# codelion/adaptive-classifier

Measured on AMD Instinct MI355X. Metric: predict() queries/sec + kNN GB/s vs HBM roofline, 768-d, higher is better.
Workload: dtype f32

## Files before the change

### adaptive-classifier_amd/csrc/attention_core.h

```cpp
#pragma once
#include "common.h"

#include <math.h>

namespace acattn {

typedef float f32x4 __attribute__((ext_vector_type(4)));
typedef float f32x16 __attribute__((ext_vector_type(16)));

__device__ __forceinline__ int crow32(int r, int h) { return (r & 3) + 8 * (r >> 2) + 4 * h; }

__device__ __forceinline__ void rope_rotate(f32x4 (&x)[8], const float* cs, const float* sn, int pos, int h) {
#pragma clang fp contract(off)
#pragma unroll
    for (int kb = 0; kb < 4; ++kb) {
        const f32x4 c = *reinterpret_cast<const f32x4*>(cs + (int64_t)pos * 32 + 8 * kb + 4 * h);
        const f32x4 s = *reinterpret_cast<const f32x4*>(sn + (int64_t)pos * 32 + 8 * kb + 4 * h);
        const f32x4 lo = x[kb], hi = x[kb + 4];
        x[kb] = lo * c + (-hi) * s;
        x[kb + 4] = hi * c + lo * s;
    }
}

template <bool ROPE, int DHT, bool FP32_OUT = true>
__device__ __forceinline__ void attention_tile(const float* qb, const float* kb_, const float* vb, int64_t ld, int S, int qt, int lane,
                                               float scale, const int64_t* mask_row, const float* rope_cos, const float* rope_sin,
                                               int window, float* ctx_rows, int H, uint16_t* ctx_planes, int64_t rows, int64_t row0,
                                               int headcol, int f16) {
#pragma clang fp contract(off)
    static_assert(DHT == 64 || (DHT == 32 && !ROPE), "head dim 64, or 32 without RoPE");
    constexpr int NKB = DHT / 8;
    const int j = lane & 31, h = lane >> 5;
    const int qi = qt * 32 + j;
    const bool qvalid = qi < S;

    f32x4 Qf[NKB];
    {
        const float* qp = qb + (int64_t)(qvalid ? qi : S - 1) * ld + 4 * h;
#pragma unroll
        for (int kb = 0; kb < NKB; ++kb) Qf[kb] = *reinterpret_cast<const f32x4*>(qp + 8 * kb);
        if constexpr (ROPE) rope_rotate(Qf, rope_cos, rope_sin, qvalid ? qi : S - 1, h);
#pragma unroll
        for (int kb = 0; kb < NKB; ++kb) Qf[kb] = Qf[kb] * scale;
    }
    f32x16 o0, o1;
#pragma unroll
    for (int r = 0; r < 16; ++r) { o0[r] = 0.f; o1[r] = 0.f; }
    float m = -INFINITY, l = 0.f;

    f32x4 Kf[NKB];
    auto load_k = [&](int k0) {
        int kr = k0 + j; if (kr > S - 1) kr = S - 1;
        const float* kp = kb_ + (int64_t)kr * ld + 4 * h;
#pragma unroll
        for (int kb = 0; kb < NKB; ++kb) Kf[kb] = *reinterpret_cast<const f32x4*>(kp + 8 * kb);
        if constexpr (ROPE) rope_rotate(Kf, rope_cos, rope_sin, kr, h);
    };
    int kbeg = 0, kend = S;
    if (window >= 0) {
        kbeg = qt * 32 - window; kbeg = kbeg < 0 ? 0 : (kbeg / 32) * 32;
        const int last = qt * 32 + 31 + window;
        if (last + 1 < kend) kend = last + 1;
    }
    load_k(kbeg);
    for (int k0 = kbeg; k0 < kend; k0 += 32) {
        const int kj = k0 + j;
        const bool kv = kj < S && (!mask_row || mask_row[kj] != 0);
        const unsigned vmask = (unsigned)(__ballot(kv && h == 0) & 0xffffffffull);
        if (vmask == 0u) { load_k(k0 + 32); continue; }
        f32x16 st;
#pragma unroll
        for (int r = 0; r < 16; ++r) st[r] = 0.f;
#pragma unroll
        for (int kb = 0; kb < NKB; ++kb)
#pragma unroll
            for (int s4 = 0; s4 < 4; ++s4)
                st = __builtin_amdgcn_mfma_f32_32x32x2f32(Kf[kb][s4], Qf[kb][s4], st, 0, 0, 0);
        load_k(k0 + 32);
        float cmax = -INFINITY;
#pragma unroll
        for (int r = 0; r < 16; ++r) {
            bool ok = (vmask >> crow32(r, h)) & 1u;
            if (window >= 0) { const int dk = qi - (k0 + crow32(r, h)); ok = ok && dk <= window && -dk <= window; }
            st[r] = ok ? st[r] : -INFINITY;
            cmax = fmaxf(cmax, st[r]);
        }
        cmax = fmaxf(cmax, __shfl_xor(cmax, 32));
        const float m_new = fmaxf(m, cmax);
        const bool none = m_new == -INFINITY;
        constexpr float kLog2e = 1.4426950408889634f;
        const float corr = none ? 1.f : __builtin_amdgcn_exp2f((m - m_new) * kLog2e);
        float psum = 0.f;
        float p[16];
#pragma unroll
        for (int r = 0; r < 16; ++r) { p[r] = none ? 0.f : __builtin_amdgcn_exp2f((st[r] - m_new) * kLog2e); psum += p[r]; }
        psum += __shfl_xor(psum, 32);
        l = __builtin_fmaf(l, corr, psum);
        m = m_new;
#pragma unroll
        for (int r = 0; r < 16; ++r) { o0[r] *= corr; o1[r] *= corr; }
#pragma unroll
        for (int r = 0; r < 16; ++r) {
            int vr = k0 + crow32(r, h); if (vr > S - 1) vr = S - 1;
            const float* vp = vb + (int64_t)vr * ld + j;
            o0 = __builtin_amdgcn_mfma_f32_32x32x2f32(vp[0], p[r], o0, 0, 0, 0);
            if constexpr (DHT == 64) o1 = __builtin_amdgcn_mfma_f32_32x32x2f32(vp[32], p[r], o1, 0, 0, 0);
        }
    }
    if (qvalid) {
        const float inv = l > 0.f ? 1.f / l : 0.f;
        if (!FP32_OUT || ctx_planes) {
            const int64_t row = row0 + qi, plane = rows * H;
#pragma unroll
            for (int t = 0; t < DHT / 32; ++t)
#pragma unroll
                for (int g = 0; g < 4; ++g) {
                    f32x4 v;
#pragma unroll
                    for (int e = 0; e < 4; ++e) v[e] = (t ? o1[4 * g + e] : o0[4 * g + e]) * inv;
                    ac::emit_planes4(ctx_planes + ac::plane_off(rows, row, headcol + 32 * t + 8 * g + 4 * h), plane, v, f16);
                }
        } else if constexpr (FP32_OUT) {
            float* dst = ctx_rows + (int64_t)qi * H;
#pragma unroll
            for (int r = 0; r < 16; ++r) {
                dst[crow32(r, h)] = o0[r] * inv;
                if constexpr (DHT == 64) dst[32 + crow32(r, h)] = o1[r] * inv;
            }
        }
    }
}

}
```

### adaptive-classifier_amd/csrc/gemm_pipe.hip

```cpp
#include "common.h"
#include "gemm_common.h"
#include "grid_sync.h"
#include "attention_core.h"

#include <stdio.h>
#include <stdlib.h>

#include <atomic>
#include <type_traits>

namespace {
using namespace acg;

constexpr int PSBK = 16;

struct PipeParams {
    const uint16_t* Ap; int64_t a_rows;
    const uint16_t* Wp; int64_t w_rows;
    float* C; int64_t ldc;
    int M, N, K;
    Epilogue epi;
    LnFuse ln;
    AttnFuse at;
    unsigned long long* stamps;
    int krot;
};

template <int STRIDE = 4>
__device__ __forceinline__ void stamp(const PipeParams& prm, int wave, int i) {
    if (prm.stamps && wave == 0) {
        const unsigned long long t = clock64();
        if ((threadIdx.x & 63) == 0) prm.stamps[(size_t)blockIdx.x * STRIDE + i] = t;
    }
}

template <int N> __device__ __forceinline__ void wait_vm() {
    static_assert(N >= 0 && N <= 63, "vmcnt immediate");
    asm volatile("s_waitcnt vmcnt(%0)" ::"n"(N) : "memory");
}

template <int TM, int TN, int WMW, int WNW, int NS, int AR = 3> struct PipeGeom {
    static constexpr int BM = 32 * TM * WMW, BN = 32 * TN * WNW;
    static constexpr int RA = BM / 32, RW = BN / 32, RG = RA + RW;
    static constexpr int NP = AR * RG;
    static constexpr int NW = WMW * WNW;
    static constexpr int PPW = (NP + NW - 1) / NW;
    static constexpr int SLOT = AR * RG * 64;
    static constexpr int LDS_BYTES = NS * SLOT * 16;
    static constexpr int TR_BYTES = NW * kTrFloats * 4;
    static constexpr int BPC_LDS = (160 * 1024) / (LDS_BYTES > TR_BYTES ? LDS_BYTES : TR_BYTES);
    static constexpr int BPC = BPC_LDS < 1 ? 1 : (BPC_LDS * NW > 16 ? (16 / NW < 1 ? 1 : 16 / NW) : BPC_LDS);
    static constexpr int WAVES_PER_SIMD = (BPC * NW + 3) / 4;
};

template <int TM, int TN, int WMW, int WNW>
__device__ __forceinline__ void ln_prefetch_residual(float (&res)[TM * TN * 16], const PipeParams& prm, int m0, int n0, int wm,
                                                     int wn, int lane) {
#pragma unroll
    for (int mi = 0; mi < TM; ++mi)
#pragma unroll
        for (int ni = 0; ni < TN; ++ni) {
            const int col = n0 + wn * (32 * TN) + ni * 32 + (lane & 31);
            const int64_t rbase = m0 + wm * (32 * TM) + mi * 32;
#pragma unroll
            for (int r = 0; r < 16; ++r) {
                int64_t row = rbase + acc_row32(r, lane);
                if (row > prm.M - 1) row = prm.M - 1;
                res[(mi * TN + ni) * 16 + r] = prm.epi.residual[row * prm.epi.ldr + col];
            }
        }
}

template <int TM, int TN, int WMW, int WNW, int AR>
__device__ __forceinline__ void store_tile_ln(f32x16 (&acc)[TM][TN], const float (&res)[TM * TN * 16], const PipeParams& prm,
                                              int bm, int bn, int ntn, int wm, int wn, int lane, int tid, int wave, float* lds_f) {
    constexpr int BM = 32 * TM * WMW, BN = 32 * TN * WNW, NW = WMW * WNW, WC = 32 * TN;
    static_assert(BM <= 64 * NW, "one thread per tile row in the combine steps");
    const Epilogue& e = prm.epi;
    const LnFuse& ln = prm.ln;
    float2* wstat = reinterpret_cast<float2*>(lds_f + NW * kTrFloats);
    float2* rstat = wstat + WNW * BM;
    unsigned* okf = reinterpret_cast<unsigned*>(rstat + BM);
    const int m0 = bm * BM, n0 = bn * BN, c = lane & 31;
#pragma unroll
    for (int mi = 0; mi < TM; ++mi)
#pragma unroll
        for (int ni = 0; ni < TN; ++ni) {
            const float bias = e.bias[n0 + wn * WC + ni * 32 + c];
#pragma unroll
            for (int r = 0; r < 16; ++r) acc[mi][ni][r] = (acc[mi][ni][r] + bias) + res[(mi * TN + ni) * 16 + r];
        }
#pragma unroll
    for (int mi = 0; mi < TM; ++mi)
#pragma unroll
        for (int r = 0; r < 16; ++r) {
            float s = 0.f;
#pragma unroll
            for (int ni = 0; ni < TN; ++ni) s += acc[mi][ni][r];
            s = acp::row16_sum(s);
            s += __shfl_xor(s, 16);
            const float mw = s * (1.0f / WC);
            float q = 0.f;
#pragma unroll
            for (int ni = 0; ni < TN; ++ni) { const float d = acc[mi][ni][r] - mw; q = fmaf(d, d, q); }
            q = acp::row16_sum(q);
            q += __shfl_xor(q, 16);
            if (c == r) wstat[wn * BM + wm * (32 * TM) + mi * 32 + acc_row32(r, lane)] = make_float2(mw, q);
        }
    __syncthreads();
    if (tid < BM) {
        float mean = 0.f;
#pragma unroll
        for (int w = 0; w < WNW; ++w) mean += wstat[w * BM + tid].x;
        mean *= 1.0f / WNW;
        float m2 = 0.f;
#pragma unroll
        for (int w = 0; w < WNW; ++w) { const float2 pw = wstat[w * BM + tid]; const float d = pw.x - mean; m2 += fmaf((float)WC * d, d, pw.y); }
        const unsigned long long bits = (unsigned long long)__float_as_uint(mean) | ((unsigned long long)__float_as_uint(m2) << 32);
        __hip_atomic_store(reinterpret_cast<unsigned long long*>(ln.part + ((size_t)bm * ntn + bn) * BM + tid), bits,
                           __ATOMIC_RELAXED, __HIP_MEMORY_SCOPE_AGENT);
    }
    asm volatile("s_waitcnt vmcnt(0)" ::: "memory");
    __syncthreads();
    if (tid == 0) {
        if (ln.fences) __hip_atomic_fetch_add(ln.count + bm, 1u, __ATOMIC_RELEASE, __HIP_MEMORY_SCOPE_AGENT);
        else __hip_atomic_fetch_add(ln.count + bm, 1u, __ATOMIC_RELAXED, __HIP_MEMORY_SCOPE_AGENT);
    }
    if (tid < 64) {
        unsigned ok = 1;
        for (long spins = 0;; ++spins) {
            const unsigned v = __hip_atomic_load(ln.count + bm, __ATOMIC_RELAXED, __HIP_MEMORY_SCOPE_AGENT);
            if (v >= (unsigned)(ntn + ln.starve)) {
                if (ln.fences) __builtin_amdgcn_fence(__ATOMIC_ACQUIRE, "agent");
                else asm volatile("" ::: "memory");
                break;
            }
            __builtin_amdgcn_s_sleep(1);
            if ((spins & 63) == 63 && (spins > (1l << 20) || __hip_atomic_load(ln.abort_, __ATOMIC_RELAXED, __HIP_MEMORY_SCOPE_AGENT))) {
                if (lane == 0) __hip_atomic_store(ln.abort_, 1u, __ATOMIC_RELAXED, __HIP_MEMORY_SCOPE_AGENT);
                ok = 0;
                break;
            }
        }
        if (lane == 0) *okf = ok;
    }
    __syncthreads();
    if (tid < BM) {
        float2 pj[8];
        const float* base = reinterpret_cast<const float*>(ln.part + (size_t)bm * ntn * BM + tid);
#pragma unroll
        for (int j = 0; j < 8; ++j) pj[j] = j < ntn ? acp::ld2_sc1(base + (size_t)j * BM * 2) : make_float2(0.f, 0.f);
        float mean = 0.f;
#pragma unroll
        for (int j = 0; j < 8; ++j) mean += pj[j].x;
        mean /= (float)ntn;
        float m2 = 0.f;
#pragma unroll
        for (int j = 0; j < 8; ++j) if (j < ntn) { const float d = pj[j].x - mean; m2 += fmaf((float)BN * d, d, pj[j].y); }
        const float var = m2 / (float)prm.N;
        const float rstd = 1.0f / sqrtf(var + ln.eps);
        rstat[tid] = make_float2(mean, *okf ? rstd : __uint_as_float(0x7fc00000u));
    }
    __syncthreads();
#pragma unroll
    for (int mi = 0; mi < TM; ++mi)
#pragma unroll
        for (int ni = 0; ni < TN; ++ni) {
            const int col = n0 + wn * WC + ni * 32 + c;
            const float g = ln.gamma[col], b = ln.beta[col];
#pragma unroll
            for (int r = 0; r < 16; ++r) {
                const float2 st = rstat[wm * (32 * TM) + mi * 32 + acc_row32(r, lane)];
                acc[mi][ni][r] = (acc[mi][ni][r] - st.x) * st.y * g + b;
            }
        }
    store_tile<EPI_IDENT, TM, BM, TN>(acc, prm.C, prm.ldc, prm.M, prm.N, m0, n0, wm, wn, lane, e);
    if (ln.planes)
        store_tile_planes<EPI_IDENT, TM, TN, AR>(acc, ln.planes, prm.M, prm.N, m0, n0, wm, wn, lane, e, lds_f + wave * kTrFloats);
}

constexpr int kAtLd = 196;
constexpr int kAtRows = 160;
constexpr int kAtCu = ac::kQkvAttnCu;
constexpr int kAtBytes = kAtRows * kAtLd * 4 + kAtCu * 4;

template <int TM, int TN, int WMW, int WNW, int AR>
__device__ __forceinline__ void qkv_attention_epilogue(f32x16 (&acc)[TM][TN], const PipeParams& prm, int bm, int head, int wm, int wn,
                                                       int lane, int wave, float* T, int cu_pref, const float (&bias)[TN]) {
    static_assert(TM == 2 && TN == 3 && WMW == 4 && WNW == 2, "built for the 256 x 192 tile (8 waves of 64 x 96)");
    constexpr int BM = 256, NW = WMW * WNW;
    const AttnFuse& at = prm.at;
    const int m0 = bm * BM, H = at.H, c = lane & 31;
    const int stride = at.smax <= 32 ? 128 : 96;
    const int tile_end = m0 + BM < prm.M ? m0 + BM : prm.M;
    int* cuT = reinterpret_cast<int*>(T + kAtRows * kAtLd);
    if (wave * 64 + lane < kAtCu) cuT[wave * 64 + lane] = cu_pref;
    const int* cuL = cuT + 1;
    const bool xchg = at.exchange != nullptr;
    const __amdgpu_buffer_rsrc_t rq = acp::make_rsrc(at.qkv, 0xffffffffu);
    const int xpart = lane >> 4, xc4 = lane & 15;
    auto qkv_byte_off = [&](int row) { return (unsigned)((((int64_t)row * 3 + xpart) * H + head * 64 + 4 * xc4) * 4); };
    auto spill_rows = [&](int row_a, int row_b, int lo_r) {
        if (lane < 48)
            for (int row = row_a; row < row_b; ++row) {
                const f32x4 v = *reinterpret_cast<const f32x4*>(T + (row - m0 - lo_r) * kAtLd + xpart * 64 + 4 * xc4);
                if (xchg) __builtin_amdgcn_raw_buffer_store_b128(__builtin_bit_cast(acp::u32x4_t, v), rq, qkv_byte_off(row), 0, 16);
                else *reinterpret_cast<f32x4*>(at.qkv + (int64_t)row * (3 * H) + xpart * H + head * 64 + 4 * xc4) = v;
            }
    };
    auto pull_rows = [&](int row_a, int row_b, int lo_r) -> bool {
        unsigned* flag = at.exchange + (size_t)(bm + 1) * (prm.N / 192) + head;
        unsigned ok = 1;
        for (long spins = 0;; ++spins) {
            if (__hip_atomic_load(flag, __ATOMIC_RELAXED, __HIP_MEMORY_SCOPE_AGENT) == at.epoch) break;
            __builtin_amdgcn_s_sleep(1);
            if ((spins & 63) == 63 && (spins > (1l << 20) || __hip_atomic_load(at.abort_, __ATOMIC_RELAXED, __HIP_MEMORY_SCOPE_AGENT))) {
                if (lane == 0) __hip_atomic_store(at.abort_, 1u, __ATOMIC_RELAXED, __HIP_MEMORY_SCOPE_AGENT);
                ok = 0;
                break;
            }
        }
        if (at.fences) __builtin_amdgcn_fence(__ATOMIC_ACQUIRE, "agent");
        else asm volatile("" ::: "memory");
        if (lane < 48) {
            constexpr int RB = 8;
            for (int r0b = row_a; r0b < row_b; r0b += RB) {
                acp::u32x4_t v[RB];
#pragma unroll
                for (int u = 0; u < RB; ++u) {
                    const int row = r0b + u < row_b ? r0b + u : row_b - 1;
                    v[u] = __builtin_amdgcn_raw_buffer_load_b128(rq, qkv_byte_off(row), 0, 16);
                }
#pragma unroll
                for (int u = 0; u < RB; ++u)
                    if (r0b + u < row_b) {
                        const acp::u32x4_t w = ok ? v[u] : acp::u32x4_t{0x7fc00000u, 0x7fc00000u, 0x7fc00000u, 0x7fc00000u};
                        *reinterpret_cast<acp::u32x4_t*>(T + (r0b + u - m0 - lo_r) * kAtLd + xpart * 64 + 4 * xc4) = w;
                    }
            }
        }
        __builtin_amdgcn_fence(__ATOMIC_RELEASE, "wavefront");
        __builtin_amdgcn_wave_barrier();
        return ok != 0;
    };
    auto xstamp = [&](int i) {
#ifdef AC_QKV_ATTN_STAMPS
        if (prm.stamps && wave == 0 && lane == 0 && i < 16) prm.stamps[(size_t)blockIdx.x * 16 + i] = clock64();
#else
        (void)i;
#endif
    };
    int pass_i = 0;
    for (int lo_r = 0; lo_r < BM; lo_r += stride, ++pass_i) {
        if (m0 + lo_r >= prm.M) break;
#pragma unroll
        for (int mi = 0; mi < TM; ++mi) {
            const int rb = wm * (32 * TM) + mi * 32;
            if (rb >= lo_r && rb < lo_r + kAtRows) {
#pragma unroll
                for (int ni = 0; ni < TN; ++ni)
#pragma unroll
                    for (int r = 0; r < 16; ++r)
                        T[(rb - lo_r + acc_row32(r, lane)) * kAtLd + wn * 96 + ni * 32 + c] = acc[mi][ni][r] + bias[ni];
            }
        }
        __syncthreads();
        xstamp(4 + 3 * pass_i);
        const int nseq = cuT[0];
        const int seq_lo = m0 + lo_r;
        const int seq_hi = seq_lo + stride < tile_end ? seq_lo + stride : tile_end;
        int s0 = 0;
        {
            int hi = nseq;
            while (s0 < hi) { const int mid = (s0 + hi) >> 1; if (cuL[mid] < seq_lo) s0 = mid + 1; else hi = mid; }
        }
        if (lo_r == 0 && wave == NW - 1) {
            const int top_end = cuL[0] < tile_end ? cuL[0] : tile_end;
            spill_rows(m0, top_end, lo_r);
            if (xchg) {
                asm volatile("s_waitcnt vmcnt(0)" ::: "memory");
                if (lane == 0) {
                    if (at.fences) __hip_atomic_store(at.exchange + (size_t)bm * (prm.N / 192) + head, at.epoch, __ATOMIC_RELEASE, __HIP_MEMORY_SCOPE_AGENT);
                    else __hip_atomic_store(at.exchange + (size_t)bm * (prm.N / 192) + head, at.epoch, __ATOMIC_RELAXED, __HIP_MEMORY_SCOPE_AGENT);
                }
            }
        }
        for (int s = s0 + wave; s < nseq; s += NW) {
            const int r0 = cuL[s];
            if (r0 >= seq_hi) break;
            const int r1 = cuL[s + 1];
            bool whole = r1 <= m0 + BM;
            if (!whole && xchg) {
                pull_rows(tile_end, r1, lo_r);
                whole = true;
            }
            if (whole) {
                const float* qb = T + (r0 - seq_lo) * kAtLd;
                const int S = r1 - r0;
                for (int qt = 0; qt * 32 < S; ++qt)
                    acattn::attention_tile<false, 64, false>(qb, qb + 64, qb + 128, kAtLd, S, qt, lane, at.scale, nullptr, nullptr, nullptr, -1,
                                                             nullptr, H, at.ctx_planes, prm.M, r0, head * 64, AR == 2);
            } else {
                spill_rows(r0, tile_end, lo_r);
            }
        }
        xstamp(5 + 3 * pass_i);
        __syncthreads();
        xstamp(6 + 3 * pass_i);
    }
}

template <int EPI, int TM, int TN, int WMW, int WNW, int NS, bool C_PLANES, int PIPE, int AR = 3>
__global__ __launch_bounds__(64 * WMW * WNW, (PipeGeom<TM, TN, WMW, WNW, NS, AR>::WAVES_PER_SIMD)) void gemm_pipe_nt(PipeParams prm) {
    using G = PipeGeom<TM, TN, WMW, WNW, NS, AR>;
    static_assert(AR == 3 || AR == 2, "operand planes: 3 = bf16x3, 2 = fp16x2");
    constexpr int BM = G::BM, BN = G::BN, RA = G::RA, RG = G::RG, NP = G::NP, NW = G::NW, PPW = G::PPW, SLOT = G::SLOT;
    static_assert(PIPE == 0 || NS >= 3, "the software-pipelined loop needs a ring of >= 3 stages");
    static_assert(NS >= 2, "ring depth");
    extern __shared__ __attribute__((aligned(16))) uint4 lds[];

    const int tid = threadIdx.x, lane = tid & 63;
    const int wave = __builtin_amdgcn_readfirstlane(tid >> 6);
    const int wm = wave / WNW, wn = wave % WNW;
    const int ntn = (prm.N + BN - 1) / BN;
    const int tile = xcd_tile_id(blockIdx.x, gridDim.x);
    const int bn = tile % ntn, bm = tile / ntn;
    const int m0 = bm * BM, n0 = bn * BN;
    const int nk = prm.K / PSBK;
    stamp<(EPI == EPI_QKV_ATTN ? 16 : 4)>(prm, wave, 0);
    float lnres[EPI == EPI_BIAS_RES_LN ? TM * TN * 16 : 1];
    if constexpr (EPI == EPI_BIAS_RES_LN) ln_prefetch_residual<TM, TN, WMW, WNW>(lnres, prm, m0, n0, wm, wn, lane);
    int at_cu_pref = 0;
    float at_bias[EPI == EPI_QKV_ATTN ? TN : 1];
    if constexpr (EPI == EPI_QKV_ATTN) {
        if (tid < kAtCu) at_cu_pref = prm.at.tile_seq[(size_t)bm * kAtCu + tid];
#pragma unroll
        for (int ni = 0; ni < TN; ++ni) {
            const int col = wn * (32 * TN) + ni * 32 + (lane & 31);
            at_bias[ni] = prm.epi.bias[(col >> 6) * prm.at.H + bn * 64 + (col & 63)];
        }
    }

    const uint16_t* pp[PPW];
    const int64_t a_step = 2 * prm.a_rows * 8, w_step = 2 * prm.w_rows * 8;
    {
        const int i32 = lane & 31, kg = lane >> 5;
        const int64_t a_plane = prm.a_rows * (int64_t)prm.K, w_plane = prm.w_rows * (int64_t)prm.K;
#pragma unroll
        for (int t = 0; t < PPW; ++t) {
            const int j = (wave + NW * t) % NP, p = j / RG, g = j % RG;
            if (g < RA) {
                int row = m0 + 32 * g + i32; if (row > prm.M - 1) row = prm.M - 1;
                pp[t] = prm.Ap + p * a_plane + ((int64_t)kg * prm.a_rows + row) * 8;
            } else {
                int row;
                if constexpr (EPI == EPI_QKV_ATTN) {
                    const int gg = g - RA;
                    row = (gg >> 1) * prm.at.H + bn * 64 + (gg & 1) * 32 + i32;
                } else {
                    row = n0 + 32 * (g - RA) + i32; if (row > prm.N - 1) row = prm.N - 1;
                }
                pp[t] = prm.Wp + p * w_plane + ((int64_t)kg * prm.w_rows + row) * 8;
            }
        }
    }
    int iss = 0;
    int a_cur = prm.krot ? ((int)(blockIdx.x & 7) * nk / 8) : 0;
    if (a_cur) {
#pragma unroll
        for (int t = 0; t < PPW; ++t) pp[t] += (int64_t)a_cur * (((wave + NW * t) % NP) % RG < RA ? a_step : w_step);
    }
    const int64_t a_back = (int64_t)(nk - 1) * a_step, w_back = (int64_t)(nk - 1) * w_step;
    auto issue = [&]() {
        const int slot = iss % NS;
#pragma unroll
        for (int t = 0; t < PPW; ++t) {
            const int j = (wave + NW * t) % NP, p = j / RG, g = j % RG;
            __builtin_amdgcn_global_load_lds((glb_void_t*)pp[t], (lds_void_t*)&lds[slot * SLOT + (p * RG + g) * 64], 16, 0, 0);
        }
        const bool wrap = a_cur + 1 == nk;
        a_cur = wrap ? 0 : a_cur + 1;
        const int64_t da = wrap ? -a_back : a_step, dw = wrap ? -w_back : w_step;
#pragma unroll
        for (int t = 0; t < PPW; ++t) pp[t] += ((wave + NW * t) % NP) % RG < RA ? da : dw;
        ++iss;
    };

    f32x16 acc[TM][TN];
#pragma unroll
    for (int a = 0; a < TM; ++a)
#pragma unroll
        for (int b = 0; b < TN; ++b)
#pragma unroll
            for (int r = 0; r < 16; ++r) acc[a][b][r] = 0.f;

    using frag_t = std::conditional_t<AR == 3, bf16x8_t, f16x8_t>;
    struct Frags { frag_t a[TM][AR], b[TN][AR]; };
    auto read_frags = [&](Frags& F, int slot) {
        const uint4* base = lds + slot * SLOT + lane;
#pragma unroll
        for (int p = 0; p < AR; ++p) {
#pragma unroll
            for (int a = 0; a < TM; ++a) F.a[a][p] = __builtin_bit_cast(frag_t, base[(p * RG + TM * wm + a) * 64]);
#pragma unroll
            for (int b = 0; b < TN; ++b) F.b[b][p] = __builtin_bit_cast(frag_t, base[(p * RG + RA + TN * wn + b) * 64]);
        }
    };
    constexpr int NPROD = AR == 3 ? 6 : 3;
    auto mfmas = [&](const Frags& F) {
        constexpr int PAIRS3[6][2] = {{2, 0}, {0, 2}, {1, 1}, {1, 0}, {0, 1}, {0, 0}};
        constexpr int PAIRS2[3][2] = {{1, 0}, {0, 1}, {0, 0}};
#pragma unroll
        for (int pr = 0; pr < NPROD; ++pr)
#pragma unroll
            for (int a = 0; a < TM; ++a)
#pragma unroll
                for (int b = 0; b < TN; ++b) {
                    if constexpr (AR == 3)
                        acc[a][b] = __builtin_amdgcn_mfma_f32_32x32x16_bf16(F.a[a][PAIRS3[pr][0]], F.b[b][PAIRS3[pr][1]], acc[a][b], 0, 0, 0);
                    else
                        acc[a][b] = __builtin_amdgcn_mfma_f32_32x32x16_f16(F.a[a][PAIRS2[pr][0]], F.b[b][PAIRS2[pr][1]], acc[a][b], 0, 0, 0);
                }
    };

#pragma unroll
    for (int s = 0; s < NS - 1; ++s) issue();
    wait_vm<(NS - 2) * PPW>();
    __builtin_amdgcn_sched_barrier(0);
    __builtin_amdgcn_s_barrier();
    __builtin_amdgcn_sched_barrier(0);
    stamp<(EPI == EPI_QKV_ATTN ? 16 : 4)>(prm, wave, 1);

    if constexpr (PIPE != 0) {
        Frags F0, F1;
        read_frags(F0, 0);
        int slot = 1 % NS;
        constexpr int NREAD = AR * (TM + TN), NMFMA = NPROD * TM * TN, MPR = NMFMA / NREAD;
        static_assert(MPR >= 1, "at least one MFMA per fragment read");
#define AC_PIPE_STEP(FC, FN)                                                                                     \
        do {                                                                                                     \
            wait_vm<(NS - 3) * PPW>();                         \
            __builtin_amdgcn_sched_barrier(0);                                                                   \
            __builtin_amdgcn_s_barrier();                 \
            __builtin_amdgcn_sched_barrier(0);                                                                   \
            issue();                                           \
            read_frags(FN, slot);                                                   \
            slot = slot + 1 == NS ? 0 : slot + 1;                                                                \
            mfmas(FC);                                                                               \
            if (PIPE == 2) {                              \
                _Pragma("unroll") for (int g_ = 0; g_ < NREAD; ++g_) {                                           \
                    __builtin_amdgcn_sched_group_barrier(0x008, MPR, 0);                                         \
                    __builtin_amdgcn_sched_group_barrier(0x100, 1, 0);                                           \
                }                                                                                                \
            }                                                                                                    \
        } while (0)
        for (int s = 0; s < nk; s += 2) {
            AC_PIPE_STEP(F0, F1);
            AC_PIPE_STEP(F1, F0);
        }
#undef AC_PIPE_STEP
    } else {
        int slot = 0;
        for (int s = 0; s < nk; ++s) {
            if (s > 0) {
                wait_vm<(NS - 2) * PPW>();
                __builtin_amdgcn_sched_barrier(0);
                __builtin_amdgcn_s_barrier();
                __builtin_amdgcn_sched_barrier(0);
            }
            issue();
            Frags F;
            read_frags(F, slot);
            slot = slot + 1 == NS ? 0 : slot + 1;
            mfmas(F);
        }
    }
    wait_vm<0>();
    stamp<(EPI == EPI_QKV_ATTN ? 16 : 4)>(prm, wave, 2);
    if constexpr (AR == 2) {
#pragma unroll
        for (int a = 0; a < TM; ++a)
#pragma unroll
            for (int b = 0; b < TN; ++b)
#pragma unroll
                for (int r = 0; r < 16; ++r) acc[a][b][r] *= ac::kF16OutScale;
    }
    if constexpr (EPI == EPI_BIAS_RES_LN) {
        __builtin_amdgcn_sched_barrier(0);
        __builtin_amdgcn_s_barrier();
        __builtin_amdgcn_sched_barrier(0);
        store_tile_ln<TM, TN, WMW, WNW, AR>(acc, lnres, prm, bm, bn, ntn, wm, wn, lane, tid, wave, reinterpret_cast<float*>(lds));
    } else if constexpr (EPI == EPI_QKV_ATTN) {
        __builtin_amdgcn_sched_barrier(0);
        __builtin_amdgcn_s_barrier();
        __builtin_amdgcn_sched_barrier(0);
        if constexpr (EPI == EPI_QKV_ATTN)
            qkv_attention_epilogue<TM, TN, WMW, WNW, AR>(acc, prm, bm, bn, wm, wn, lane, wave, reinterpret_cast<float*>(lds), at_cu_pref, at_bias);
    } else if (C_PLANES) {
        __builtin_amdgcn_sched_barrier(0);
        __builtin_amdgcn_s_barrier();
        __builtin_amdgcn_sched_barrier(0);
        store_tile_planes<EPI, TM, TN, AR>(acc, reinterpret_cast<uint16_t*>(prm.C), prm.M, prm.N, m0, n0, wm, wn, lane, prm.epi,
                                       reinterpret_cast<float*>(lds) + wave * kTrFloats);
    } else {
        store_tile<EPI, TM, BM, TN>(acc, prm.C, prm.ldc, prm.M, prm.N, m0, n0, wm, wn, lane, prm.epi);
    }
    if (prm.stamps) { wait_vm<0>(); stamp<(EPI == EPI_QKV_ATTN ? 16 : 4)>(prm, wave, 3); }
}

std::atomic<int> g_krot{-1};
int krot_enabled() {
    int v = g_krot.load(std::memory_order_relaxed);
    if (v < 0) {
        const char* e = getenv("AC_GEMM_KROT");
        v = (e && atoi(e) != 0) ? 1 : 0;
        g_krot.store(v, std::memory_order_relaxed);
    }
    return v;
}
unsigned long long* g_stamps = nullptr;
int64_t g_stamp_cap = 0;

template <int EPI, int TM, int TN, int WMW, int WNW, int NS, bool CP, int PIPE, int AR = 3>
int launch_one(PipeParams p, hipStream_t stream) {
    using G = PipeGeom<TM, TN, WMW, WNW, NS, AR>;
    static_assert(G::BM == 32 * TM * WMW && G::BN == 32 * TN * WNW && G::NW == WMW * WNW, "gemm_plan.h derives a ring cfg's grid and block from its digits");
    const int64_t tiles = (int64_t)((p.M + G::BM - 1) / G::BM) * ((p.N + G::BN - 1) / G::BN);
    constexpr int LN_BYTES = G::TR_BYTES + (WNW + 1) * G::BM * 8 + 16;
    const size_t lds = EPI == EPI_BIAS_RES_LN ? (size_t)(G::LDS_BYTES > LN_BYTES ? G::LDS_BYTES : LN_BYTES)
                     : EPI == EPI_QKV_ATTN    ? (size_t)(G::LDS_BYTES > kAtBytes ? G::LDS_BYTES : kAtBytes)
                                              : (size_t)(G::LDS_BYTES > G::TR_BYTES || !CP ? G::LDS_BYTES : G::TR_BYTES);
    static std::atomic<unsigned long long> attr_set{0};
    if (ac::first_call_on_device(attr_set))
        AC_HIP_CHECK(hipFuncSetAttribute((const void*)gemm_pipe_nt<EPI, TM, TN, WMW, WNW, NS, CP, PIPE, AR>,
                                         hipFuncAttributeMaxDynamicSharedMemorySize, (int)lds));
    const char* se = g_stamps ? getenv("AC_GEMM_STAMP_EPI") : nullptr;
    const char* sk = g_stamps ? getenv("AC_GEMM_STAMP_K") : nullptr;
    p.stamps = (g_stamps && tiles <= g_stamp_cap && (!se || atoi(se) == EPI) && (!sk || atoi(sk) == p.K)) ? g_stamps : nullptr;
    p.krot = krot_enabled();
    hipLaunchKernelGGL((gemm_pipe_nt<EPI, TM, TN, WMW, WNW, NS, CP, PIPE, AR>), dim3((unsigned)tiles), dim3(64 * WMW * WNW), lds, stream, p);
    AC_LAUNCH_CHECK();
    return AC_OK;
}

template <int TM, int TN, int WMW, int WNW, int NS, int PIPE, int AR = 3>
int launch_cfg(int cls, bool cp, const PipeParams& p, hipStream_t stream) {
    if (cp && cls == EPI_BIAS_GELU) return launch_one<EPI_BIAS_GELU, TM, TN, WMW, WNW, NS, true, PIPE, AR>(p, stream);
    if (cp && cls == EPI_BIAS) return launch_one<EPI_BIAS, TM, TN, WMW, WNW, NS, true, PIPE, AR>(p, stream);
    if constexpr (TN == 2 && AR == 3) if (cp && cls == EPI_GEGLU32) return launch_one<EPI_GEGLU32, TM, TN, WMW, WNW, NS, true, PIPE>(p, stream);
    if (!cp && cls == EPI_BIAS) return launch_one<EPI_BIAS, TM, TN, WMW, WNW, NS, false, PIPE, AR>(p, stream);
    if (!cp && cls == EPI_BIAS_RES) return launch_one<EPI_BIAS_RES, TM, TN, WMW, WNW, NS, false, PIPE, AR>(p, stream);
    if constexpr (TM == 1 && TN == 2 && WMW == 4 && WNW == 2 && NS == 6 && PIPE == 2)
        if (!cp && cls == EPI_BIAS_RES_LN) return launch_one<EPI_BIAS_RES_LN, TM, TN, WMW, WNW, NS, false, PIPE, AR>(p, stream);
    ac::set_error("gemm_pipe: epilogue class %d (planes out %d) not built for %s", cls, (int)cp, AR == 2 ? "fp16x2 operands" : "this tile");
    return AC_EUNSUPPORTED;
}

}

extern "C" int ac_gemm_set_krot(int on) {
    AC_TEST_HOOK_ONLY("ac_gemm_set_krot");
    g_krot.store(on ? 1 : 0, std::memory_order_relaxed);
    return AC_OK;
}
extern "C" int ac_gemm_debug_stamps(unsigned long long* d_buf, int64_t capacity_workgroups) {
    AC_TEST_HOOK_ONLY("ac_gemm_debug_stamps");
    g_stamps = d_buf;
    g_stamp_cap = d_buf ? capacity_workgroups : 0;
    return AC_OK;
}

namespace ac {

#define AC_PIPE_CONFIGS(X)                                                                         \
    X(2, 2, 2, 2, 3, 2)        \
    X(1, 2, 4, 2, 6, 1) X(1, 2, 4, 2, 6, 2)  \
    X(2, 2, 4, 2, 4, 2)                               \
    X(2, 3, 4, 2, 3, 2)                               \
    X(3, 2, 2, 4, 3, 2)                               \
    X(2, 4, 4, 2, 3, 2)

#define AC_PIPE_CONFIGS_F16(X)                                                                     \
    X(2, 4, 4, 2, 4, 2)                                           \
    X(2, 3, 4, 2, 4, 2)                                                    \
    X(2, 2, 4, 2, 6, 2)                                                    \
    X(1, 2, 4, 2, 8, 2)

int launch_gemm_pipe(int cfg, const uint16_t* Ap, int64_t a_rows, const uint16_t* Wp, int64_t w_rows, float* C, int64_t ldc,
                     uint16_t* Cp, int M, int N, int K, int cls, const acg::Epilogue& epi, hipStream_t stream, int f16) {
    PipeParams p{};
    p.Ap = Ap; p.a_rows = a_rows; p.Wp = Wp; p.w_rows = w_rows;
    p.C = Cp ? reinterpret_cast<float*>(Cp) : C; p.ldc = ldc; p.M = M; p.N = N; p.K = K; p.epi = epi;
    const bool cp = Cp != nullptr;
#define AC_CASE(TM, TN, WMW, WNW, NS, PIPE) \
    if (!f16 && cfg == (((((TM * 10 + TN) * 10 + WMW) * 10 + WNW) * 10 + NS) * 10 + PIPE)) return launch_cfg<TM, TN, WMW, WNW, NS, PIPE>(cls, cp, p, stream);
    AC_PIPE_CONFIGS(AC_CASE)
#undef AC_CASE
#define AC_CASE(TM, TN, WMW, WNW, NS, PIPE) \
    if (f16 && cfg == (((((TM * 10 + TN) * 10 + WMW) * 10 + WNW) * 10 + NS) * 10 + PIPE)) return launch_cfg<TM, TN, WMW, WNW, NS, PIPE, 2>(cls, cp, p, stream);
    AC_PIPE_CONFIGS(AC_CASE)
    AC_PIPE_CONFIGS_F16(AC_CASE)
#undef AC_CASE
    set_error("gemm_pipe: configuration %d not built", cfg);
    return AC_EUNSUPPORTED;
}


bool ln_fusion_enabled();
static int exchange_fences() {
    static const int v = [] { const char* e = getenv("AC_EXCHANGE_FENCES"); return e && atoi(e) != 0 ? 1 : 0; }();
    return v;
}
static std::atomic<long long> g_qkv_attn_launches{0};
bool qkv_attn_applies(int M, int H, int heads, int smax) {
    if (const char* e = getenv("AC_QKV_ATTN_FUSION"); e && atoi(e) == 0) return false;
    return qkv_attn_shape(M, H, heads, smax, gemm_env());
}
__global__ __launch_bounds__(kAtCu) void qkv_attn_tile_seq_kernel(const int32_t* __restrict__ cu, int b, int ntiles, int32_t* __restrict__ out) {
    const int t = blockIdx.x, i = threadIdx.x;
    auto first_at_or_after = [&](int row) { int lo = 0, hi = b; while (lo < hi) { const int mid = (lo + hi) >> 1; if (cu[mid] < row) lo = mid + 1; else hi = mid; } return lo; };
    const int sb = first_at_or_after(t * kQkvAttnRows), se = first_at_or_after((t + 1) * kQkvAttnRows), n = se - sb;
    int v = 0;
    if (i == 0) v = n;
    else if (i - 1 <= n) v = cu[sb + i - 1];
    out[(size_t)t * kAtCu + i] = v;
}
size_t qkv_attn_tile_seq_bytes(int M) { return ((size_t)(M + kQkvAttnRows - 1) / kQkvAttnRows) * kAtCu * sizeof(int32_t); }
int qkv_attn_tile_seq(const int32_t* cu, int b, int M, int32_t* tile_seq, hipStream_t stream) {
    const int ntiles = (M + kQkvAttnRows - 1) / kQkvAttnRows;
    hipLaunchKernelGGL(qkv_attn_tile_seq_kernel, dim3(ntiles), dim3(kAtCu), 0, stream, cu, b, ntiles, tile_seq);
    AC_LAUNCH_CHECK();
    return AC_OK;
}
enum { OCC_LN = 0, OCC_QKV_ATTN = 1, OCC_QKV_ATTN_F16 = 2 };
static int64_t resident_capacity(int slot, const void* fn, int threads, int lds) {
    static std::atomic<int> occ_cache[3][64];
    int dev = 0;
    if (hipGetDevice(&dev) != hipSuccess || dev < 0 || dev > 63) dev = 0;
    int occ = occ_cache[slot][dev].load(std::memory_order_relaxed);
    if (occ <= 0) {
        int per_cu = 0;
        (void)hipFuncSetAttribute(fn, hipFuncAttributeMaxDynamicSharedMemorySize, lds);
        if (hipOccupancyMaxActiveBlocksPerMultiprocessor(&per_cu, fn, threads, lds) != hipSuccess) { (void)hipGetLastError(); per_cu = 0; }
        occ = per_cu > 0 ? per_cu : -1;
        occ_cache[slot][dev].store(occ, std::memory_order_relaxed);
    }
    return occ > 0 ? (int64_t)occ * dev_info().cus : 0;
}
bool qkv_attn_exchange_applies(int M, int heads, int f16) {
    if (!ln_fusion_enabled()) return false;
    if (const char* e = getenv("AC_QKV_ATTN_EXCHANGE"); e && atoi(e) == 0) return false;
    const int64_t tiles = (int64_t)((M + kQkvAttnRows - 1) / kQkvAttnRows) * heads;
    using G16 = PipeGeom<2, 3, 4, 2, 4, 2>; using G = PipeGeom<2, 3, 4, 2, 3, 3>;
    if (f16) return tiles <= resident_capacity(OCC_QKV_ATTN_F16, (const void*)gemm_pipe_nt<EPI_QKV_ATTN, 2, 3, 4, 2, 4, false, 2, 2>, 64 * G16::NW,
                                               G16::LDS_BYTES > kAtBytes ? G16::LDS_BYTES : kAtBytes);
    return tiles <= resident_capacity(OCC_QKV_ATTN, (const void*)gemm_pipe_nt<EPI_QKV_ATTN, 2, 3, 4, 2, 3, false, 2, 3>, 64 * G::NW,
                                      G::LDS_BYTES > kAtBytes ? G::LDS_BYTES : kAtBytes);
}
int launch_gemm_pipe_qkv_attn(const uint16_t* Ap, int64_t a_rows, const uint16_t* Wp, int64_t w_rows, const float* bias, int M, int H,
                              int heads, const int32_t* cu, const int32_t* tile_seq, int b, int smax, float scale, uint16_t* ctx_planes,
                              float* qkv, hipStream_t stream, int f16, unsigned* exchange, unsigned epoch, unsigned* abort_flag) {
    AC_REQUIRE(qkv_attn_applies(M, H, heads, smax), AC_EUNSUPPORTED, "gemm_pipe: fused attention epilogue not applicable (M %d H %d heads %d longest %d)",
               M, H, heads, smax);
    AC_REQUIRE(Ap && Wp && bias && cu && tile_seq && ctx_planes && qkv && b >= 1, AC_EINVAL, "gemm_pipe_qkv_attn: null pointer");
    PipeParams p{};
    p.Ap = Ap; p.a_rows = a_rows; p.Wp = Wp; p.w_rows = w_rows; p.C = qkv; p.ldc = 3 * (int64_t)H; p.M = M; p.N = 3 * H; p.K = H;
    p.epi.bias = bias;
    p.at.cu = cu; p.at.tile_seq = tile_seq; p.at.b = b; p.at.H = H; p.at.smax = smax; p.at.scale = scale; p.at.ctx_planes = ctx_planes;
    p.at.qkv = qkv;
    AC_REQUIRE(!exchange || (abort_flag && qkv_attn_exchange_applies(M, heads, f16)), AC_EINVAL,
               "gemm_pipe_qkv_attn: the in-launch exchange needs every tile resident (%d rows x %d heads) and an abort word", M, heads);
    p.at.exchange = exchange; p.at.epoch = epoch; p.at.abort_ = abort_flag; p.at.fences = exchange_fences();
    g_qkv_attn_launches.fetch_add(1, std::memory_order_relaxed);
    return f16 ? launch_one<EPI_QKV_ATTN, 2, 3, 4, 2, 4, false, 2, 2>(p, stream)
               : launch_one<EPI_QKV_ATTN, 2, 3, 4, 2, 3, false, 2, 3>(p, stream);
}

static std::atomic<int> g_ln_fusion{-1};
static std::atomic<long long> g_ln_launches{0};
bool ln_fusion_enabled() {
    if (const int o = call_opts().ln_fusion; o >= 0) return o != 0;
    int v = g_ln_fusion.load(std::memory_order_relaxed);
    if (v < 0) {
        const char* e = getenv("AC_LN_FUSION");
        v = (e && atoi(e) == 0) ? 0 : 1;
        g_ln_fusion.store(v, std::memory_order_relaxed);
    }
    return v != 0;
}
static int64_t ln_resident_capacity() {
    using G = PipeGeom<1, 2, 4, 2, 6, 3>;
    constexpr int LN_BYTES = G::TR_BYTES + (2 + 1) * G::BM * 8 + 16;
    return resident_capacity(OCC_LN, (const void*)gemm_pipe_nt<EPI_BIAS_RES_LN, 1, 2, 4, 2, 6, false, 2, 3>, 64 * G::NW,
                             G::LDS_BYTES > LN_BYTES ? G::LDS_BYTES : LN_BYTES);
}
bool pipe_ln_applies(int M, int N, int K) {
    return ln_fusion_enabled() && pipe_ln_shape(M, N, K, gemm_env()) && tiles_of(M, N, kLnBM, kLnBN) <= ln_resident_capacity();
}
size_t pipe_ln_part_bytes(int M, int N) { return (size_t)((M + kLnBM - 1) / kLnBM) * (size_t)(N / kLnBN) * kLnBM * sizeof(float2); }
int pipe_ln_panels(int M) { return (M + kLnBM - 1) / kLnBM; }

int launch_gemm_pipe_ln(const uint16_t* Ap, int64_t a_rows, const uint16_t* Wp, int64_t w_rows, const float* bias,
                        const float* residual, int64_t ldr, float* C, int64_t ldc, int M, int N, int K, const float* gamma,
                        const float* beta, float eps, void* part, unsigned* count, unsigned* abort_flag, uint16_t* planes,
                        hipStream_t stream, int f16) {
    AC_REQUIRE(pipe_ln_applies(M, N, K), AC_EUNSUPPORTED, "gemm_pipe: fused LayerNorm epilogue not applicable to %d x %d x %d", M, N, K);
    AC_REQUIRE(Ap && Wp && bias && residual && C && gamma && beta && part && count && abort_flag, AC_EINVAL, "gemm_pipe_ln: null pointer");
    PipeParams p{};
    p.Ap = Ap; p.a_rows = a_rows; p.Wp = Wp; p.w_rows = w_rows; p.C = C; p.ldc = ldc; p.M = M; p.N = N; p.K = K;
    p.epi.bias = bias; p.epi.residual = residual; p.epi.ldr = ldr;
    p.ln.gamma = gamma; p.ln.beta = beta; p.ln.eps = eps; p.ln.part = (float2*)part; p.ln.count = count; p.ln.abort_ = abort_flag;
    p.ln.fences = exchange_fences();
    p.ln.planes = planes; p.ln.starve = (call_opts().ln_fusion >= 0 ? call_opts().ln_fusion : g_ln_fusion.load(std::memory_order_relaxed)) == 2 ? 1 : 0;
    g_ln_launches.fetch_add(1, std::memory_order_relaxed);
    return f16 ? launch_cfg<1, 2, 4, 2, 6, 2, 2>(EPI_BIAS_RES_LN, false, p, stream)
               : launch_cfg<1, 2, 4, 2, 6, 2>(EPI_BIAS_RES_LN, false, p, stream);
}
}

extern "C" int ac_gemm_set_ln_fusion(int on) {
    AC_TEST_HOOK_ONLY("ac_gemm_set_ln_fusion");
    ac::g_ln_fusion.store(on == 2 ? 2 : (on ? 1 : 0), std::memory_order_relaxed);
    return AC_OK;
}

extern "C" int64_t ac_gemm_ln_fusion_launches(void) { return (int64_t)ac::g_ln_launches.load(std::memory_order_relaxed); }
extern "C" int64_t ac_gemm_qkv_attn_launches(void) { return (int64_t)ac::g_qkv_attn_launches.load(std::memory_order_relaxed); }

static int parse_pipe_table(const char* spec, acg::PipeTable* t) {
    if (!spec) { t->n = -1; return AC_OK; }
    int n = 0;
    const char* p = spec;
    while (*p && n < 16) {
        int N = 0, K = 0, cfg = 0, used = 0;
        if (sscanf(p, "%dx%d=%d%n", &N, &K, &cfg, &used) != 3) { ac::set_error("gemm pipe table: cannot parse '%s'", p); return AC_EINVAL; }
        t->rules[n++] = {N, K, cfg};
        p += used;
        if (*p == ';') ++p;
    }
    t->n = n;
    return AC_OK;
}
extern "C" int ac_gemm_set_pipe_table(const char* spec) {
    AC_TEST_HOOK_ONLY("ac_gemm_set_pipe_table");
    return parse_pipe_table(spec, &ac::g_pipe_table);
}
extern "C" int ac_gemm_set_pipe_table_f16(const char* spec) {
    AC_TEST_HOOK_ONLY("ac_gemm_set_pipe_table_f16");
    return parse_pipe_table(spec, &ac::g_pipe_table_f16);
}
```

Measured before the change: 52700.

## Skip masked PV MFMAs, batch V loads, and idle dead waves in fused GEMM

The attention tile now skips P·V MFMAs and V loads for key rows that are fully masked or outside the window, and batches V loads ahead of their MFMAs in groups of eight. It also stops prefetching K past the loop end, and adds an option to load K in the current iteration rather than one ahead, which the fused QKV-attention path uses. In the pipelined GEMM, waves whose M rows fall entirely past the matrix end only issue loads and take part in barriers, skipping fragment reads and MFMAs. This adds branching and a wave-uniform readfirstlane on the live mask, and the dead-wave loops must stay barrier-matched with the main loop.

```diff
diff --git a/adaptive-classifier_amd/csrc/attention_core.h b/adaptive-classifier_amd/csrc/attention_core.h
--- a/adaptive-classifier_amd/csrc/attention_core.h
+++ b/adaptive-classifier_amd/csrc/attention_core.h
@@ -22,7 +22,7 @@
     }
 }
 
-template <bool ROPE, int DHT, bool FP32_OUT = true>
+template <bool ROPE, int DHT, bool FP32_OUT = true, bool K_AHEAD = true>
 __device__ __forceinline__ void attention_tile(const float* qb, const float* kb_, const float* vb, int64_t ld, int S, int qt, int lane,
                                                float scale, const int64_t* mask_row, const float* rope_cos, const float* rope_sin,
                                                int window, float* ctx_rows, int H, uint16_t* ctx_planes, int64_t rows, int64_t row0,
@@ -62,12 +62,16 @@
         const int last = qt * 32 + 31 + window;
         if (last + 1 < kend) kend = last + 1;
     }
-    load_k(kbeg);
+    if constexpr (K_AHEAD) load_k(kbeg);
     for (int k0 = kbeg; k0 < kend; k0 += 32) {
+        if constexpr (!K_AHEAD) load_k(k0);
         const int kj = k0 + j;
         const bool kv = kj < S && (!mask_row || mask_row[kj] != 0);
         const unsigned vmask = (unsigned)(__ballot(kv && h == 0) & 0xffffffffull);
-        if (vmask == 0u) { load_k(k0 + 32); continue; }
+        if (vmask == 0u) {
+            if constexpr (K_AHEAD) if (k0 + 32 < kend) load_k(k0 + 32);
+            continue;
+        }
         f32x16 st;
 #pragma unroll
         for (int r = 0; r < 16; ++r) st[r] = 0.f;
@@ -76,7 +80,7 @@
 #pragma unroll
             for (int s4 = 0; s4 < 4; ++s4)
                 st = __builtin_amdgcn_mfma_f32_32x32x2f32(Kf[kb][s4], Qf[kb][s4], st, 0, 0, 0);
-        load_k(k0 + 32);
+        if constexpr (K_AHEAD) if (k0 + 32 < kend) load_k(k0 + 32);
         float cmax = -INFINITY;
 #pragma unroll
         for (int r = 0; r < 16; ++r) {
@@ -99,12 +103,33 @@
         m = m_new;
 #pragma unroll
         for (int r = 0; r < 16; ++r) { o0[r] *= corr; o1[r] *= corr; }
+        unsigned live = vmask;
+        if (window >= 0) {
+            const int lo = qt * 32 - window - k0, hi = qt * 32 + 31 + window - k0;
+            if (lo > 0) live &= lo < 32 ? 0xffffffffu << lo : 0u;
+            if (hi < 31) live &= hi >= 0 ? 0xffffffffu >> (31 - hi) : 0u;
+        }
+        live = (unsigned)__builtin_amdgcn_readfirstlane((int)(live | (live >> 4)));
+        constexpr int PVC = 8;
 #pragma unroll
-        for (int r = 0; r < 16; ++r) {
-            int vr = k0 + crow32(r, h); if (vr > S - 1) vr = S - 1;
-            const float* vp = vb + (int64_t)vr * ld + j;
-            o0 = __builtin_amdgcn_mfma_f32_32x32x2f32(vp[0], p[r], o0, 0, 0, 0);
-            if constexpr (DHT == 64) o1 = __builtin_amdgcn_mfma_f32_32x32x2f32(vp[32], p[r], o1, 0, 0, 0);
+        for (int rb = 0; rb < 16; rb += PVC) {
+            float v0[PVC], v1[PVC];
+#pragma unroll
+            for (int u = 0; u < PVC; ++u) {
+                const int r = rb + u;
+                if (!((live >> crow32(r, 0)) & 1u)) continue;
+                int vr = k0 + crow32(r, h); if (vr > S - 1) vr = S - 1;
+                const float* vp = vb + (int64_t)vr * ld + j;
+                v0[u] = vp[0];
+                if constexpr (DHT == 64) v1[u] = vp[32];
+            }
+#pragma unroll
+            for (int u = 0; u < PVC; ++u) {
+                const int r = rb + u;
+                if (!((live >> crow32(r, 0)) & 1u)) continue;
+                o0 = __builtin_amdgcn_mfma_f32_32x32x2f32(v0[u], p[r], o0, 0, 0, 0);
+                if constexpr (DHT == 64) o1 = __builtin_amdgcn_mfma_f32_32x32x2f32(v1[u], p[r], o1, 0, 0, 0);
+            }
         }
     }
     if (qvalid) {
diff --git a/adaptive-classifier_amd/csrc/gemm_pipe.hip b/adaptive-classifier_amd/csrc/gemm_pipe.hip
--- a/adaptive-classifier_amd/csrc/gemm_pipe.hip
+++ b/adaptive-classifier_amd/csrc/gemm_pipe.hip
@@ -298,7 +298,7 @@
                 const float* qb = T + (r0 - seq_lo) * kAtLd;
                 const int S = r1 - r0;
                 for (int qt = 0; qt * 32 < S; ++qt)
-                    acattn::attention_tile<false, 64, false>(qb, qb + 64, qb + 128, kAtLd, S, qt, lane, at.scale, nullptr, nullptr, nullptr, -1,
+                    acattn::attention_tile<false, 64, false, false>(qb, qb + 64, qb + 128, kAtLd, S, qt, lane, at.scale, nullptr, nullptr, nullptr, -1,
                                                              nullptr, H, at.ctx_planes, prm.M, r0, head * 64, AR == 2);
             } else {
                 spill_rows(r0, tile_end, lo_r);
@@ -431,7 +431,28 @@
     __builtin_amdgcn_sched_barrier(0);
     stamp<(EPI == EPI_QKV_ATTN ? 16 : 4)>(prm, wave, 1);
 
-    if constexpr (PIPE != 0) {
+    const bool dead_wave = m0 + 32 * TM * wm >= prm.M;
+    if (__builtin_expect(dead_wave, 0)) {
+        if constexpr (PIPE != 0) {
+            for (int s = 0; s < nk; ++s) {
+                wait_vm<(NS - 3) * PPW>();
+                __builtin_amdgcn_sched_barrier(0);
+                __builtin_amdgcn_s_barrier();
+                __builtin_amdgcn_sched_barrier(0);
+                issue();
+            }
+        } else {
+            for (int s = 0; s < nk; ++s) {
+                if (s > 0) {
+                    wait_vm<(NS - 2) * PPW>();
+                    __builtin_amdgcn_sched_barrier(0);
+                    __builtin_amdgcn_s_barrier();
+                    __builtin_amdgcn_sched_barrier(0);
+                }
+                issue();
+            }
+        }
+    } else if constexpr (PIPE != 0) {
         Frags F0, F1;
         read_frags(F0, 0);
         int slot = 1 % NS;
```

Result: faster. 53420 (median of 6 runs) (+1.4%).
